# francois-rozet/sda

Hardware: AMD Instinct MI355X
Metric: diffusion-steps/s (Kolmogorov 64x256x256 posterior sampling; unit = one predictor-corrector step of a 16-trajectory per-GPU shard) (higher is better)
Workload: dtype f32; 1 GPU; kolmogorov256; per_gpu_batch=16, global_batch=16, guided=True, corrections=1, schedule_steps=1000, hipgraph_step=True, observation=fused Subsample (hand-written adjoint; no autograd through A), corrector_noise=row-keyed Philox (sda_randn_rows), parallelism=dp1 (batch-sharded, no in-loop collective), ranks_seen=1, process_group_live=False

## Files before the change

include/sda_hip.h:

```cpp
#ifndef SDA_HIP_H
#define SDA_HIP_H

#include <stdint.h>

#ifdef __cplusplus
extern "C" {
#endif

#define SDA_ABI_VERSION 13

enum {
    SDA_OK = 0,
    SDA_E_BADARG = -1,
    SDA_E_UNSUPPORTED = -2,
    SDA_E_LDS = -3
};

enum { SDA_ACT_NONE = 0, SDA_ACT_SILU = 1, SDA_ACT_RELU = 2, SDA_ACT_ELU = 3, SDA_ACT_GELU = 4, SDA_ACT_SELU = 5 };

int sda_abi_version(void);

typedef struct sda_conv_desc {
    const float* x;
    int64_t x_sn_outer, x_sn_inner;
    int32_t n_inner;
    int32_t x_n_off;
    int64_t x_sc, x_sy, x_sx;
    int32_t cx;
    const float* ctx;
    int64_t ctx_sn;
    int32_t cctx;
    int32_t n;
    int32_t hs, ws;
    int32_t up_h, up_w;
    int32_t zins_h, zins_w;
    const float* mod;
    int64_t mod_sn;
    const float* ln_mean;
    const float* ln_rstd;
    int32_t act_in;
    int32_t kh, kw, stride_h, stride_w, circular;
    const float* w;
    int32_t cin_pad, cout_pad;
    const float* bias;
    float* out;
    int32_t cout, ho, wo;
    const float* dact_z;
    int32_t act_d;
    const float* res;
    int32_t mt;
    const float* w_wino;
    int32_t explicit_pad, pad_h, pad_w;
    int64_t out_sn, out_sc, out_sy, out_sx;
    const float* w_wino4;
    int32_t pool_h, pool_w;
    const float* w_wino4_zp;
    const void* w_h2;
    float w_h2_scale;
    float x_amax_static;
    const float* x_amax;
    float* out_amax;
} sda_conv_desc;

int sda_conv_igemm(const sda_conv_desc* d, void* stream);
int sda_conv_parity4(const sda_conv_desc* d, void* stream);
int sda_conv_igemm_path(const sda_conv_desc* d);
int64_t sda_conv_igemm_lds_bytes(const sda_conv_desc* d);

typedef struct sda_block1d_desc {
    int32_t n, c, len;
    int32_t circular, act, unbiased;
    float eps;
    int32_t k_pad, m_pad;
    const float* a;
    const float* mod;
    int64_t mod_sn;
    const float* w1; const float* b1;
    const float* w2; const float* b2;
    float* z;
    float* mean; float* rstd;
    float* y;
    const float* g;
    float* gx;
} sda_block1d_desc;
int sda_block1d_fwd(const sda_block1d_desc* d, void* stream);
int sda_block1d_bwd(const sda_block1d_desc* d, void* stream);

#define SDA_NET1D_MAXB 8
typedef struct sda_net1d_desc {
    int32_t n, len;
    int32_t cin, c, cout;
    int32_t nblocks;
    int32_t circular, act, unbiased;
    float eps;
    const float* x; int64_t x_sn, x_sc, x_sx;
    float* out; int64_t out_sn, out_sc, out_sx;
    const float* w;
    const float* bias;
    const float* mod[SDA_NET1D_MAXB];
    int64_t mod_sn;
    float* a_save; float* z_save; int64_t save_stride;
    float* mean_save; float* rstd_save; int64_t stat_stride;
} sda_net1d_desc;
int sda_net1d_fwd(const sda_net1d_desc* d, void* stream);
int sda_net1d_bwd(const sda_net1d_desc* d, void* stream);

typedef struct sda_net1d_fuse {
    float cx0, cx1, cn;
    const float* coef;
    const float* y; int64_t y_sn;
    int32_t p_start, p_step, p_stop;
    int32_t c_start, c_step, c_stop;
    float std, gamma;
    float* ghat;
    const float* eps;
    int32_t mode;
    float* xs;
    const float* step_coef;
    float* partial; int32_t partial_stride;
} sda_net1d_fuse;
int sda_net1d_fwd_fused(const sda_net1d_desc* d, const sda_net1d_fuse* f, void* stream);
int sda_net1d_bwd_fused(const sda_net1d_desc* d, const sda_net1d_fuse* f, void* stream);
int sda_net1d_tiles(const sda_net1d_desc* d);

int sda_step1d_prologue(const float* table, int row_len, int64_t* istep, const float* t_dev, int nt,
                        int alpha_kind, float eta, float k, int sigma_kind,
                        const float* freqs, int nf, const float* w0, const float* b0, int hidden, const float* w2, const float* b2, int e,
                        const float* wp, const float* bp, int cp,
                        float* out_coef, int64_t* out_step, float* mod, void* stream);
int sda_pc_correct_keyed(float* x, const float* eps, int b, int64_t per_sample, const float* partial, int nchunk, float tau,
                         float sigma, const float* coef_dev, uint64_t seed, int64_t row0, const int64_t* draw_dev, int64_t draw_mul,
                         int64_t draw_add, void* stream);

int sda_pack_conv_weight(const float* w, int cout, int cin, int kh, int kw, int transpose, int cin_keep,
                         float* dst, int k_pad, int m_pad, void* stream);

int sda_pack_conv_weight_wino(const float* w, int cout, int cin, int transpose, int cin_keep, float* dst, int k_pad,
                              int m_pad, void* stream);

int sda_pack_conv_weight_wino4(const float* w, int cout, int cin, int transpose, int cin_keep, float* dst, int k_pad,
                               int m_pad, void* stream);
int sda_pack_conv_weight_wino4_zp(const float* w_wino4, int k_pad, int m_pad, float* dst, void* stream);
int64_t sda_wino4_zp_floats(int k_pad, int m_pad);

int sda_ln_stats(const float* x, int n, int c, int hw, const float* mod, int64_t mod_sn, float eps, int unbiased,
                 float* mean, float* rstd, void* stream);
int sda_ln_apply(const float* x, int n, int c, int hw, const float* mod, int64_t mod_sn, const float* mean,
                 const float* rstd, float* y, void* stream);
int sda_ln_bwd(const float* gh, const float* x, int n, int c, int h, int w, const float* mod, int64_t mod_sn,
               const float* mean, const float* rstd, int unbiased, int pool_h, int pool_w, const float* res, float* gx,
               void* stream);
int sda_ln_bwd_amax(const float* gh, const float* x, int n, int c, int h, int w, const float* mod, int64_t mod_sn,
                    const float* mean, const float* rstd, int unbiased, int pool_h, int pool_w, const float* res, float* gx,
                    float* amax, void* stream);

int sda_time_embed(const float* t, int nt, const float* freqs, int nf, const float* w0, const float* b0, int hidden,
                   const float* w2, const float* b2, int e, float* emb, void* stream);
int sda_linear_small(const float* x, int rows, int in_f, const float* w, const float* b, int out_f, float* y,
                     void* stream);

int sda_linear(const float* x, int rows, int in_f, const float* w, const float* b, int out_f, int trans_w, int act_in,
               int act_out, const float* dact_z, int act_d, const float* res, float* y, void* stream);
int sda_row_ln(const float* x, int rows, int f, float eps, int unbiased, float* y, float* mean, float* rstd, void* stream);
int sda_row_ln_bwd(const float* gh, const float* x, int rows, int f, const float* mean, const float* rstd, int unbiased,
                   const float* res, float* gx, void* stream);

#define SDA_MLP_MAXG 32
typedef struct sda_mlp_desc {
    int32_t rows, ngemm;
    int32_t act, unbiased;
    float eps;
    int32_t kind[SDA_MLP_MAXG];
    int32_t in_f[SDA_MLP_MAXG], out_f[SDA_MLP_MAXG];
    int32_t w_off[SDA_MLP_MAXG], b_off[SDA_MLP_MAXG];
    const float* w; const float* bias;
    const float* x; int64_t x_ld;
    float* out; int64_t out_ld;
    float* a_save; float* z_save; int64_t save_stride; int32_t save_ld;
    float* mean_save; float* rstd_save; int64_t stat_stride;
} sda_mlp_desc;
int sda_mlp_fwd(const sda_mlp_desc* d, void* stream);
int sda_mlp_bwd(const sda_mlp_desc* d, void* stream);
int sda_mlp_slab_floats(int in_f, int out_f);

typedef struct sda_mlp_win {
    int32_t nw, len, c, emb_n;
    const float* x; const float* emb;
    float cx0, cx1, cn;
    const float* coef;
    const float* y; int64_t y_sn;
    int32_t p_start, p_step, p_stop, c_start, c_step, c_stop;
    float std, gamma;
    float* eps; float* ghat;
    float* gwin;
} sda_mlp_win;
int sda_mlp_fwd_win(const sda_mlp_desc* d, const sda_mlp_win* w, void* stream);
// ... 84 lines not shown
```

sda_amd/_lib.py:

```python
import ctypes
import os
from ctypes import POINTER, Structure, c_float, c_int, c_int32, c_int64, c_uint32, c_uint64, c_void_p

import torch

HERE = os.path.dirname(os.path.abspath(__file__))
LIB_PATH = os.environ.get('SDA_HIP_LIB') or os.path.join(HERE, 'lib', 'libsda_hip.so')

ACT_IDS = {None: 0, 'none': 0, 'SiLU': 1, 'ReLU': 2, 'ELU': 3, 'GELU': 4, 'SELU': 5}

c_fp = c_void_p


class ConvDesc(Structure):
    _fields_ = [
        ('x', c_fp),
        ('x_sn_outer', c_int64), ('x_sn_inner', c_int64),
        ('n_inner', c_int32),
        ('x_n_off', c_int32),
        ('x_sc', c_int64), ('x_sy', c_int64), ('x_sx', c_int64),
        ('cx', c_int32),
        ('ctx', c_fp),
        ('ctx_sn', c_int64),
        ('cctx', c_int32),
# ... 94 lines not shown
        ('a_save', c_fp), ('z_save', c_fp), ('save_stride', c_int64), ('save_ld', c_int32),
        ('mean_save', c_fp), ('rstd_save', c_fp), ('stat_stride', c_int64),
    ]


class MlpWin(Structure):
    _fields_ = [
        ('nw', c_int32), ('len', c_int32), ('c', c_int32), ('emb_n', c_int32),
        ('x', c_fp), ('emb', c_fp),
        ('cx0', c_float), ('cx1', c_float), ('cn', c_float),
        ('coef', c_fp),
        ('y', c_fp), ('y_sn', c_int64),
        ('p_start', c_int32), ('p_step', c_int32), ('p_stop', c_int32),
        ('c_start', c_int32), ('c_step', c_int32), ('c_stop', c_int32),
        ('std', c_float), ('gamma', c_float),
        ('eps', c_fp), ('ghat', c_fp),
        ('gwin', c_fp),
    ]


class Net1dFuse(Structure):
    _fields_ = [
        ('cx0', c_float), ('cx1', c_float), ('cn', c_float),
        ('coef', c_fp),
        ('y', c_fp), ('y_sn', c_int64),
        ('p_start', c_int32), ('p_step', c_int32), ('p_stop', c_int32),
        ('c_start', c_int32), ('c_step', c_int32), ('c_stop', c_int32),
        ('std', c_float), ('gamma', c_float),
        ('ghat', c_fp),
        ('eps', c_fp),
        ('mode', c_int32),
        ('xs', c_fp),
        ('step_coef', c_fp),
        ('partial', c_fp), ('partial_stride', c_int32),
    ]


SIGNATURES = {
    'sda_abi_version': (c_int, []),
    'sda_conv_igemm': (c_int, [POINTER(ConvDesc), c_void_p]),
    'sda_gauss_cotangent': (c_int, [c_void_p, c_int64, c_void_p, c_int64, c_float, c_float, c_float, c_float, c_void_p, c_void_p, c_void_p]),
    'sda_block1d_fwd': (c_int, [POINTER(Block1dDesc), c_void_p]),
    'sda_block1d_bwd': (c_int, [POINTER(Block1dDesc), c_void_p]),
    'sda_net1d_fwd': (c_int, [POINTER(Net1dDesc), c_void_p]),
    'sda_net1d_bwd': (c_int, [POINTER(Net1dDesc), c_void_p]),
    'sda_net1d_fwd_fused': (c_int, [POINTER(Net1dDesc), POINTER(Net1dFuse), c_void_p]),
    'sda_net1d_bwd_fused': (c_int, [POINTER(Net1dDesc), POINTER(Net1dFuse), c_void_p]),
    'sda_net1d_tiles': (c_int, [POINTER(Net1dDesc)]),
    'sda_step1d_prologue': (c_int, [c_fp, c_int, c_fp, c_fp, c_int, c_int, c_float, c_float, c_int, c_fp, c_int, c_fp, c_fp, c_int,
                                    c_fp, c_fp, c_int, c_fp, c_fp, c_int, c_fp, c_fp, c_fp, c_void_p]),
    'sda_pc_correct_keyed': (c_int, [c_fp, c_fp, c_int, c_int64, c_fp, c_int, c_float, c_float, c_fp, c_uint64, c_int64, c_fp, c_int64,
                                     c_int64, c_void_p]),
    'sda_conv_parity4': (c_int, [POINTER(ConvDesc), c_void_p]),
    'sda_conv_igemm_path': (c_int, [POINTER(ConvDesc)]),
    'sda_conv_igemm_lds_bytes': (c_int64, [POINTER(ConvDesc)]),
    'sda_pack_conv_weight': (c_int, [c_fp, c_int, c_int, c_int, c_int, c_int, c_int, c_fp, c_int, c_int, c_void_p]),
    'sda_pack_conv_weight_wino': (c_int, [c_fp, c_int, c_int, c_int, c_int, c_fp, c_int, c_int, c_void_p]),
    'sda_pack_conv_weight_wino4': (c_int, [c_fp, c_int, c_int, c_int, c_int, c_fp, c_int, c_int, c_void_p]),
    'sda_pack_conv_weight_wino4_zp': (c_int, [c_fp, c_int, c_int, c_fp, c_void_p]),
    'sda_wino4_zp_floats': (c_int64, [c_int, c_int]),
    'sda_ln_stats': (c_int, [c_fp, c_int, c_int, c_int, c_fp, c_int64, c_float, c_int, c_fp, c_fp, c_void_p]),
    'sda_ln_apply': (c_int, [c_fp, c_int, c_int, c_int, c_fp, c_int64, c_fp, c_fp, c_fp, c_void_p]),
    'sda_ln_bwd': (c_int, [c_fp, c_fp, c_int, c_int, c_int, c_int, c_fp, c_int64, c_fp, c_fp, c_int, c_int, c_int, c_fp, c_fp,
                           c_void_p]),
    'sda_ln_bwd_amax': (c_int, [c_fp, c_fp, c_int, c_int, c_int, c_int, c_fp, c_int64, c_fp, c_fp, c_int, c_int, c_int, c_fp, c_fp,
                           c_fp, c_void_p]),
    'sda_time_embed': (c_int, [c_fp, c_int, c_fp, c_int, c_fp, c_fp, c_int, c_fp, c_fp, c_int, c_fp, c_void_p]),
    'sda_linear_small': (c_int, [c_fp, c_int, c_int, c_fp, c_fp, c_int, c_fp, c_void_p]),
    'sda_linear': (c_int, [c_fp, c_int, c_int, c_fp, c_fp, c_int, c_int, c_int, c_int, c_fp, c_int, c_fp, c_fp, c_void_p]),
    'sda_mlp_fwd': (c_int, [POINTER(MlpDesc), c_void_p]),
    'sda_mlp_bwd': (c_int, [POINTER(MlpDesc), c_void_p]),
    'sda_mlp_slab_floats': (c_int, [c_int, c_int]),
    'sda_mlp_fwd_win': (c_int, [POINTER(MlpDesc), POINTER(MlpWin), c_void_p]),
    'sda_mlp_bwd_win': (c_int, [POINTER(MlpDesc), POINTER(MlpWin), c_void_p]),
    'sda_mc_finish': (c_int, [c_fp, c_fp, c_fp, c_int, c_int, c_int, c_int, c_float, c_float, c_fp, c_int, c_fp, c_fp, c_fp, c_fp, c_void_p]),
    'sda_row_ln': (c_int, [c_fp, c_int, c_int, c_float, c_int, c_fp, c_fp, c_fp, c_void_p]),
    'sda_row_ln_bwd': (c_int, [c_fp, c_fp, c_int, c_int, c_fp, c_fp, c_int, c_fp, c_fp, c_void_p]),
    'sda_obs_subsample': (c_int, [c_fp, POINTER(c_int), POINTER(c_int), POINTER(c_int), POINTER(c_int), c_fp, c_void_p]),
    'sda_obs_subsample_adjoint': (c_int, [c_fp, POINTER(c_int), POINTER(c_int), POINTER(c_int), POINTER(c_int), c_fp, c_void_p]),
    'sda_obs_pointwise': (c_int, [c_fp, c_int64, c_int, c_fp, c_void_p]),
    'sda_obs_pointwise_vjp': (c_int, [c_fp, c_fp, c_int64, c_int, c_fp, c_void_p]),
    'sda_obs_mask': (c_int, [c_fp, c_int64, c_fp, c_int64, c_fp, c_void_p]),
    'sda_obs_timediff': (c_int, [c_fp, c_int64, c_int, c_int64, c_int, c_int, c_fp, c_void_p]),
    'sda_obs_timediff_adjoint': (c_int, [c_fp, c_int64, c_int, c_int64, c_int, c_int, c_fp, c_void_p]),
    'sda_obs_subsample_guidance': (c_int, [c_fp, c_fp, c_fp, c_int64, POINTER(c_int), POINTER(c_int), POINTER(c_int), POINTER(c_int),
                                           c_float, c_float, c_float, c_float, c_fp, c_fp, c_void_p]),
    'sda_obs_coarsen': (c_int, [c_fp, c_int64, c_int, c_int, c_int, c_fp, c_void_p]),
    'sda_obs_coarsen_adjoint': (c_int, [c_fp, c_int64, c_int, c_int, c_int, c_fp, c_void_p]),
    'sda_obs_vorticity': (c_int, [c_fp, c_int64, c_int, c_int, c_fp, c_void_p]),
    'sda_obs_vorticity_adjoint': (c_int, [c_fp, c_int64, c_int, c_int, c_fp, c_void_p]),
    'sda_fold': (c_int, [c_fp, c_int, c_int, c_int, c_int, c_int, c_fp, c_void_p]),
    'sda_fold_adjoint': (c_int, [c_fp, c_int, c_int, c_int, c_int, c_int, c_fp, c_void_p]),
    'sda_unfold_adjoint': (c_int, [c_fp, c_int, c_int, c_int, c_int, c_int, c_int64, c_fp, c_void_p]),
    'sda_vp_schedule': (c_int, [c_fp, c_int, c_float, c_float, c_int, c_fp, c_void_p]),
    'sda_pc_predict': (c_int, [c_fp, c_fp, c_int64, c_float, c_float, c_fp, c_void_p]),
    'sda_sumsq_partial': (c_int, [c_fp, c_int, c_int64, c_fp, c_int, c_void_p]),
    'sda_pc_correct': (c_int, [c_fp, c_fp, c_fp, c_int, c_int64, c_fp, c_int, c_float, c_float, c_fp, c_void_p]),
    'sda_randn_rows': (c_int, [c_fp, c_int, c_int64, c_uint64, c_int64, c_int64, c_fp, c_int64, c_int64, c_void_p]),
    'sda_clock_probe': (c_int, [c_void_p, c_int, c_void_p, c_int, c_void_p]),
    'sda_conv_h2': (c_int, [POINTER(ConvDesc), c_void_p]),
    'sda_conv_h2_supported': (c_int, [POINTER(ConvDesc)]),
    'sda_pack_conv_weight_h2': (c_int, [c_fp, c_int, c_int, c_int, c_float, c_void_p, c_void_p]),
    'sda_conv_h2_packed_bytes': (c_int64, [c_int, c_int, c_int]),
    'sda_pack_conv_weight_h2_up': (c_int, [c_fp, c_int, c_int, c_float, c_void_p, c_void_p]),
    'sda_conv_h2_up_packed_bytes': (c_int64, [c_int, c_int]),
    'sda_pack_conv_weight_h2_rows': (c_int, [c_fp, c_int, c_int, c_int, c_float, c_void_p, c_void_p]),
# ... 54 lines not shown
```

sda_amd/build.py:

```python
import hashlib
import os
import subprocess
import sys

HERE = os.path.dirname(os.path.abspath(__file__))
CSRC = os.path.join(HERE, 'csrc')
LIBDIR = os.environ.get('SDA_LIBDIR') or os.path.join(HERE, 'lib')
ARCH = 'gfx950'
SOURCES = ['conv_igemm.hip', 'conv_wino.hip', 'conv_wino4.hip', 'conv_small1d.hip', 'conv_few.hip', 'conv_par4.hip', 'conv_h2.hip', 'conv3d.hip', 'block1d.hip', 'net1d.hip', 'step1d.hip', 'norm.hip', 'elementwise.hip', 'linear.hip', 'mlp1d.hip', 'observe.hip', 'metrics.hip', 'noise.hip', 'probe.hip']
HIPCC = os.environ.get('HIPCC', '/opt/rocm/bin/hipcc')
EXTRA_FLAGS = os.environ.get('SDA_EXTRA_HIPCC_FLAGS', '').split()
CONV_PARTS = 4


def _digest(deps, flags=()):
    h = hashlib.sha256()
    for d in deps:
        h.update(os.path.basename(d).encode())
        with open(d, 'rb') as f:
            h.update(f.read())
    h.update(' '.join(flags).encode())
    return h.hexdigest()


def _newer(target, deps, flags=()):
    stamp = target + '.stamp'
    if not os.path.exists(target) or not os.path.exists(stamp):
        return True
    with open(stamp) as f:
        return f.read().strip() != _digest(deps, flags)


def _stamp(target, deps, flags=()):
    with open(target + '.stamp', 'w') as f:
        f.write(_digest(deps, flags))


def _headers():
    hs = [os.path.join(CSRC, f) for f in os.listdir(CSRC) if f.endswith('.hpp')]
    hs.append(os.path.join(os.path.dirname(HERE), 'include', 'sda_hip.h'))
    return hs


def build(force=False, verbose=False):
    os.makedirs(LIBDIR, exist_ok=True)
    objs = []
    hdrs = _headers()
    procs = []
    units = []
    for src in SOURCES:
        if src == 'conv_igemm.hip':
            units += [(src, f'_p{k}', [f'-DSDA_CONV_PART={k}']) for k in range(CONV_PARTS)]
        else:
            units.append((src, '', []))
    for src, suffix, flags in units:
        sp = os.path.join(CSRC, src)
        if not os.path.exists(sp):
            continue
        obj = os.path.join(LIBDIR, src.replace('.hip', suffix + '.o'))
        objs.append(obj)
        cflags = ['-O3', '-std=c++17', '-fPIC', '-ffp-contract=off'] + flags + EXTRA_FLAGS
        if force or _newer(obj, [sp] + hdrs, cflags):
# ... 37 lines not shown
```

sda_amd/engine.py:

```python
import math
from dataclasses import dataclass
from typing import List, Optional

import torch
import torch.nn as nn
from torch import Tensor

from . import ops
from ._lib import SdaHipError
from .ops import PackedConv, conv_out_size, make_conv_desc


def _lib_net1d_maxb() -> int:
    from ._lib import NET1D_MAXB
    return NET1D_MAXB


def _net1d_span_ok(sc: int, sx: int, channels: int, length: int) -> bool:
    return sc >= 0 and sx >= 0 and sc * channels + sx * length < 1 << 30


CHUNK_HBM_FRACTION = 0.45
KEEP_HBM_FRACTION = 0.45
PARITY_SPLIT = True
# ... 8 lines not shown
    hs: int
    ws: int
    sn_outer: int
    sc: int
    sy: int
    sx: int
    sn_inner: int = 0
    n_inner: int = 1
    ctx: Optional[Tensor] = None
    cctx: int = 0
    ctx_sn: int = 0


def planar_source(a: Tensor) -> dict:
    n, c, h, w = a.shape
    return dict(x_ptr=a.data_ptr(), n=n, cx=c, hs=h, ws=w, x_sn_outer=c * h * w, x_sc=h * w, x_sy=w, x_sx=1)


class _ConvCache:

    def __init__(self, conv: nn.Module):
        if conv.dilation != (1,) * len(conv.dilation) or conv.groups != 1:
            raise NotImplementedError('dilated / grouped convolutions have no gfx950 kernel')
        if conv.padding_mode not in ('zeros', 'circular'):
            raise NotImplementedError(f"padding_mode={conv.padding_mode!r} (supported: 'zeros', 'circular')")
        ks = conv.kernel_size
        if any(k % 2 == 0 for k in ks):
            raise NotImplementedError('even kernel sizes are not supported')
        self.conv = conv
        self.kh, self.kw = (1, ks[0]) if len(ks) == 1 else ks
        st = conv.stride
        self.sh, self.sw = (1, st[0]) if len(st) == 1 else st
        self.circular = conv.padding_mode == 'circular'
        self.cin, self.cout = conv.in_channels, conv.out_channels
        self._key = None
        self._fwd = None
        self._bwd = {}
        self._parity = None

    def _sync(self):
        w = self.conv.weight
        key = (w.data_ptr(), ops.tensor_version(w), str(w.device), None if self.conv.bias is None else ops.tensor_version(self.conv.bias),
               ops.MULTIPLY)
        if key != self._key:
            self._key, self._fwd, self._bwd, self._parity = key, None, {}, None

    def invalidate(self):
        self._key = None

    def fwd(self) -> PackedConv:
        self._sync()
        if self._fwd is None:
            self._fwd = PackedConv(self.conv.weight, self.conv.bias, transpose=False)
        return self._fwd

    def bwd(self, cin_keep: Optional[int] = None) -> PackedConv:
        self._sync()
        if cin_keep not in self._bwd:
            self._bwd[cin_keep] = PackedConv(self.conv.weight, None, transpose=True, cin_keep=cin_keep)
        return self._bwd[cin_keep]

    def bwd_parity(self):
        self._sync()
        if self._parity is None:
            taps = []
            for k, s in ((self.kh, self.sh), (self.kw, self.sw)):
                if s == 1:
                    taps.append([(None, list(range(k)), k // 2)])
                elif s == 2 and k == 3:
                    taps.append([(0, [1], 0), (1, [0, 2], 0)])
                else:
                    taps = None
                    break
            if taps is None or (self.sh == 1 and self.sw == 1):
                self._parity = False
            else:
                w = self.conv.weight.detach()
                if w.dim() == 3:
                    w = w.unsqueeze(2)
                out = []
                for py, ty, ph in taps[0]:
                    for px, tx, pw in taps[1]:
                        sub = w[:, :, ty][:, :, :, tx].contiguous()
                        out.append((py, px, PackedConv(sub, None, transpose=True), (ph, pw)))
                self._parity = out
        return self._parity or None

    def bwd_parity4(self):
        classes = self.bwd_parity()
        if not classes or len(classes) != 4 or [(py, px) for py, px, _, _ in classes] != [(0, 0), (0, 1), (1, 0), (1, 1)]:
            return None
        if getattr(self, '_parity4', None) is None or self._parity4[0] is not classes:
            pks = [pk for _, _, pk, _ in classes]
            if any(pk.k_pad != pks[0].k_pad or pk.m_pad != pks[0].m_pad or pk.m_pad != pk.m_real for pk in pks):
                return None
            self._parity4 = (classes, torch.cat([pk.packed for pk in pks]))
        return self._parity4[1]


def launch_conv(pk: PackedConv, src: dict, out: Tensor, ho: int, wo: int, *, circular: bool, stride=(1, 1), up=(1, 1),
                zins=(1, 1), bias: Optional[Tensor] = None, mod: Optional[Tensor] = None, mod_sn: int = 0,
                ln=None, act_in: int = 0, dact_z: Optional[Tensor] = None, act_d: int = 0, res: Optional[Tensor] = None,
                ctx: Optional[Tensor] = None, cctx: int = 0, ctx_sn: int = 0, pad=None, parity4_w: Optional[Tensor] = None,
                pool=(1, 1), x_amax=None, out_amax: Optional[Tensor] = None, h2_only: bool = False):
    out_strides = (0, 0, 0, 0)
    if not out.is_contiguous():
        out_strides = tuple(out.stride())
        for t in (dact_z, res):
            if t is not None and tuple(t.stride()) != out_strides:
                raise SdaHipError('conv epilogue operands must share the layout of the output view')
    zp = pk.wino4_zp() if (tuple(up) == (2, 2) or tuple(pool) == (2, 2)) and hasattr(pk, 'wino4_zp') else None
    d = make_conv_desc(**src, w_ptr=pk.packed.data_ptr(), cin_pad=pk.k_pad, cout_pad=pk.m_pad, cout=pk.m_real,
                       kh=pk.kh, kw=pk.kw, out_ptr=out.data_ptr(), ho=ho, wo=wo, mt=pk.mt,
                       stride_h=stride[0], stride_w=stride[1], circular=circular, up_h=up[0], up_w=up[1],
                       zins_h=zins[0], zins_w=zins[1],
                       ctx_ptr=None if ctx is None else ctx.data_ptr(), cctx=cctx, ctx_sn=ctx_sn,
                       mod_ptr=None if mod is None else mod.data_ptr(), mod_sn=mod_sn,
                       ln_mean_ptr=None if ln is None else ln[0].data_ptr(),
                       ln_rstd_ptr=None if ln is None else ln[1].data_ptr(),
                       act_in=act_in, bias_ptr=None if bias is None else bias.data_ptr(),
                       dact_z_ptr=None if dact_z is None else dact_z.data_ptr(), act_d=act_d,
                       res_ptr=None if res is None else res.data_ptr(),
                       w_wino_ptr=None if getattr(pk, 'wino', None) is None else pk.wino.data_ptr(),
                       w_wino4_ptr=None if getattr(pk, 'wino4', None) is None else pk.wino4.data_ptr(),
                       pad=pad, out_strides=out_strides, pool=pool, w_wino4_zp_ptr=None if zp is None else zp.data_ptr())
    if pool != (1, 1):
        if tuple(pool) == (2, 2) and ops.H2_POOL and x_amax is not None and getattr(pk, 'h2', None) is not None:
            packing = pk.h2_pool()
            if packing is not None and ops.conv_h2(d, pk, x_amax, out_amax, packing=packing):
                return d
        return d if ops.conv_pooled(d) else None
    if getattr(pk, 'h2', None) is not None and parity4_w is None:
        bound = math.sqrt(src['cx']) if ln is not None else x_amax
        packing = None
        if tuple(up) == (2, 2):
            packing = pk.h2_up() if ops.H2_UP else None
            if packing is None:
                bound = None
        elif tuple(zins) == (2, 2) or tuple(stride) == (2, 2):
            packing = (pk.h2_zins() if tuple(zins) == (2, 2) else pk.h2_s2()) if ops.H2_S2 else None
            if packing is None:
                bound = None
        if ops.conv_h2(d, pk, bound, out_amax, packing=packing):
            return d
    if h2_only:
        return None
    if parity4_w is not None:
        d.w = parity4_w.data_ptr()
        d.kh = d.kw = 2
        return d if ops.conv_parity4(d) else None
    ops.conv_igemm(d)
    return d


class _Block:
    def __init__(self, block, width: int, mod_off: int):
        from .nn import LayerNorm, activation_id
        residue = block.residue
        if not (len(residue) == 4 and isinstance(residue[0], LayerNorm)):
            raise NotImplementedError('unexpected residue structure')
        self.ln = residue[0]
        self.conv1 = _ConvCache(residue[1])
        self.act = activation_id(residue[2])
        self.conv2 = _ConvCache(residue[3])
        self.project = block.project[0]
        self.width = width
        self.mod_off = mod_off


class _Level:
    pass


class UNetEngine:
    def __init__(self, unet):
        from .nn import LN_UNBIASED
        if unet.spatial not in (1, 2):
            raise NotImplementedError('this engine serves spatial = 1, 2 (spatial = 3: engine3d.UNet3dEngine)')
        self.unet = unet
        self.unbiased = LN_UNBIASED
        self.depth = len(unet.hidden_blocks)
        D = self.depth
        self.levels: List[_Level] = []
        off = 0
        for lvl in range(D):
            lev = _Level()
            lev.C = unet.hidden_channels[lvl]
            j = D - 1 - lvl
            head = unet.heads[lvl] if lvl == 0 else unet.heads[lvl][0]
            lev.head = _ConvCache(head)
            if lvl == 0:
                lev.tail = _ConvCache(unet.tails[j])
                lev.tail_ln = None
            else:
                lev.tail_ln = unet.tails[j][0]
                lev.tail = _ConvCache(unet.tails[j][2])
            lev.descent, lev.ascent = [], []
            for blk in unet.descent[lvl]:
                lev.descent.append(_Block(blk, lev.C, off)); off += lev.C
            for blk in unet.ascent[j]:
                lev.ascent.append(_Block(blk, lev.C, off)); off += lev.C
            self.levels.append(lev)
        self.mod_total = off
# ... 551 lines not shown
```

sda_amd/ops.py:

```python
import ctypes
import math
import os
from typing import Optional

import torch
from torch import Tensor

from . import _lib
from ._lib import ACT_IDS, ConvDesc

CONV_CK = 8
WINOGRAD = os.environ.get('SDA_CONV_WINO', '1') != '0'
WINOGRAD4 = os.environ.get('SDA_CONV_WINO4', '1') != '0'
MULTIPLY = os.environ.get('SDA_MULTIPLY', 'f32')
if MULTIPLY not in ('f32', 'f16x2'):
    raise ValueError(f"SDA_MULTIPLY={MULTIPLY!r} (expected 'f32' or 'f16x2')")


def set_multiply(mode: str) -> str:
    global MULTIPLY
    if mode not in ('f32', 'f16x2'):
        raise ValueError(f"multiply mode {mode!r} (expected 'f32' or 'f16x2')")
    prev, MULTIPLY = MULTIPLY, mode
    return prev
# ... 165 lines not shown
    if packing is None:
        desc.w_h2, desc.w_h2_scale = pk.h2.data_ptr(), pk.h2_scale
    else:
        desc.w_h2, desc.w_h2_scale = packing[0].data_ptr(), packing[1]
    if torch.is_tensor(x_amax):
        desc.x_amax, desc.x_amax_static = x_amax.data_ptr(), 0.0
    else:
        desc.x_amax, desc.x_amax_static = None, float(x_amax)
    desc.out_amax = None if out_amax is None else out_amax.data_ptr()
    if not lib.sda_conv_h2_supported(ctypes.byref(desc)):
        desc.w_h2 = None
        return False
    prof = conv_profile
    if prof is not None:
        e0, e1 = torch.cuda.Event(enable_timing=True), torch.cuda.Event(enable_timing=True)
        e0.record()
    if out_amax is not None:
        out_amax.zero_()
    _lib.check(lib.sda_conv_h2(ctypes.byref(desc), _stream()), 'sda_conv_h2')
    if prof is not None:
        e1.record()
        fam = 'h2up' if (desc.up_h == 2 or desc.pool_h == 2) else 'h2s2' if (desc.zins_h == 2 or desc.stride_h == 2) else 'h2'
        prof.records.append((e0, e1, prof.flops(desc) / float(max(1, desc.zins_h) * max(1, desc.zins_w)), fam))
        rd, wr = prof.alg_bytes(desc)
        b = prof.family_bytes.setdefault(fam, [0.0, 0.0])
        b[0] += rd
        b[1] += wr
    return True


PARITY4 = os.environ.get('SDA_CONV_PAR4', '1') != '0'
WINO4_BM64 = os.environ.get('SDA_W4_BM64', '1') != '0'


def conv_parity4(desc: ConvDesc) -> bool:
    lib = _lib.load()
    prof = conv_profile
    if prof is not None:
        e0, e1 = torch.cuda.Event(enable_timing=True), torch.cuda.Event(enable_timing=True)
        e0.record()
    rc = lib.sda_conv_parity4(ctypes.byref(desc), _stream())
    if rc == -2:
        return False
    _lib.check(rc, 'sda_conv_parity4')
    if prof is not None:
        e1.record()
        prof.records.append((e0, e1, 2.0 * desc.n * desc.ho * desc.wo * desc.cout * desc.cx * 9, 'par4'))
        b = prof.family_bytes.setdefault('par4', [0.0, 0.0])
        b[0] += 4.0 * desc.n * desc.cx * desc.hs * desc.ws + 4.0 * 9 * desc.cx * desc.cout + (16.0 * desc.n * desc.cout * desc.ho * desc.wo if desc.res else 0.0)
        b[1] += 16.0 * desc.n * desc.cout * desc.ho * desc.wo
    return True


POOLED = os.environ.get('SDA_CONV_POOLED', '1') != '0'


def conv_pooled(desc: ConvDesc) -> bool:
    lib = _lib.load()
    if lib.sda_conv_igemm_path(ctypes.byref(desc)) < 0:
        return False
    conv_igemm(desc)
    return True


CONV_FAMILIES = ('direct', 'wino', 'wino4', 'small1d', 'few', 'wino4zp')


def conv_path(desc: ConvDesc) -> int:
    return _lib.load().sda_conv_igemm_path(ctypes.byref(desc))


def pack_conv_weight(w: Tensor, cout: int, cin: int, kh: int, kw: int, transpose: bool, keep: int, dst: Tensor,
                     k_pad: int, m_pad: int):
    _lib.check(_lib.load().sda_pack_conv_weight(w.data_ptr(), cout, cin, kh, kw, int(transpose), keep, dst.data_ptr(),
                                                k_pad, m_pad, _stream()), 'sda_pack_conv_weight')


class PackedConv:

    def __init__(self, weight: Tensor, bias: Optional[Tensor], transpose: bool = False, cin_keep: Optional[int] = None):
        _dev(weight, bias)
        w = weight.detach().contiguous()
        cout, cin = w.shape[0], w.shape[1]
        ks = tuple(w.shape[2:])
        self.kh, self.kw = (1, ks[0]) if len(ks) == 1 else ks
        self._transpose = bool(transpose)
        self._w_ref = w if (MULTIPLY == 'f16x2' and len(ks) == 2) else None
        self._h2_up = None
        self._h2_pool = None
        self._h2_zins = None
        self._h2_s2 = None
        if transpose:
            keep = cin if cin_keep is None else cin_keep
            self.k_real, self.m_real = cout, keep
        else:
            keep = cin
            self.k_real, self.m_real = cin, cout
        self.mt = pick_mt(self.m_real)
        self.k_pad = round_up(self.k_real, CONV_CK)
        self.m_pad = round_up(self.m_real, 32 * self.mt)
        self.packed = torch.empty(self.kh * self.kw * self.k_pad * self.m_pad, device=w.device, dtype=torch.float32)
        pack_conv_weight(w, cout, cin, self.kh, self.kw, transpose, keep, self.packed, self.k_pad, self.m_pad)
        self.bias = None if (bias is None or transpose) else bias.detach().contiguous()
        self.wino = None
        if WINOGRAD and (self.kh, self.kw) == (3, 3) and self.m_real % 96 == 0 and self.mt == 3:
            self.wino = torch.empty(16 * self.k_pad * self.m_pad, device=w.device, dtype=torch.float32)
            _lib.check(_lib.load().sda_pack_conv_weight_wino(w.data_ptr(), cout, cin, int(transpose), keep,
                                                             self.wino.data_ptr(), self.k_pad, self.m_pad, _stream()),
                       'sda_pack_conv_weight_wino')
        self.wino4 = None
        if WINOGRAD4 and (self.kh, self.kw) == (3, 3) and self.m_pad == self.m_real and (self.wino is not None or (WINO4_BM64 and self.m_real % 32 == 0)):
            self.wino4 = torch.empty(16 * self.k_pad * self.m_pad, device=w.device, dtype=torch.float32)
            _lib.check(_lib.load().sda_pack_conv_weight_wino4(w.data_ptr(), cout, cin, int(transpose), keep,
                                                              self.wino4.data_ptr(), self.k_pad, self.m_pad, _stream()),
                       'sda_pack_conv_weight_wino4')
        self._wino4_zp = None
        if self.wino4 is not None:
            lib = _lib.load()
            self._wino4_zp = torch.empty(int(lib.sda_wino4_zp_floats(self.k_pad, self.m_pad)), device=w.device, dtype=torch.float32)
            _lib.check(lib.sda_pack_conv_weight_wino4_zp(self.wino4.data_ptr(), self.k_pad, self.m_pad, self._wino4_zp.data_ptr(), _stream()),
                       'sda_pack_conv_weight_wino4_zp')

        self.h2 = None
        if MULTIPLY == 'f16x2' and (self.kh, self.kw) == (3, 3) and (not transpose or keep == cin) and w.numel() > 0:
            lib = _lib.load()
            nbytes = int(lib.sda_conv_h2_packed_bytes(cout, cin, int(transpose)))
            if nbytes > 0:
                w_amax = float(w.abs().max())
                if w_amax > 0.0 and math.isfinite(w_amax):
                    self.h2 = torch.empty(nbytes, device=w.device, dtype=torch.uint8)
                    _lib.check(lib.sda_pack_conv_weight_h2(w.data_ptr(), cout, cin, int(transpose), w_amax, self.h2.data_ptr(), _stream()),
                               'sda_pack_conv_weight_h2')
                    self.h2_scale = float(lib.sda_conv_h2_scale(w_amax))
                    self.out_amax = torch.zeros(1, device=w.device, dtype=torch.float32)
                    self.in_amax = torch.zeros(1, device=w.device, dtype=torch.float32)

    def _h2_wsum(self) -> Tensor:
        w = self._w_ref
        cout, cin = w.shape[0], w.shape[1]
        rows = (((0,), (1, 2)), ((0, 1), (2,)))
        wsum = torch.empty(4, cout, cin, 4, device=w.device, dtype=torch.float32)
        for py in range(2):
            for px in range(2):
                for a_ in range(2):
                    for b_ in range(2):
                        acc = None
                        for dy in rows[py][a_]:
                            for dx in rows[px][b_]:
                                acc = w[:, :, dy, dx] if acc is None else acc + w[:, :, dy, dx]
                        wsum[2 * py + px, :, :, 2 * a_ + b_] = acc
        return wsum

    def h2_up(self):
        if self.h2 is None or self._transpose or getattr(self, '_w_ref', None) is None:
            return None
        if getattr(self, '_h2_up', None) is None:
            lib = _lib.load()
            cout, cin = self._w_ref.shape[0], self._w_ref.shape[1]
            nbytes = int(lib.sda_conv_h2_up_packed_bytes(cout, cin))
            self._h2_up = False
            if nbytes > 0:
                wsum = self._h2_wsum()
# ... 485 lines not shown
```

Before: 0.1378 diffusion-steps/s.

## Add Winograd-style kernel for stride-2 3x3 forward convolutions

Adds a HIP kernel that computes stride-2 3x3 convolutions through a 5x5 transformed-input product, with weights pre-transformed into 25 positions at pack time. Producer waves stage transformed input and weight slabs into double-buffered LDS while consumer waves run f32 MFMA accumulations, and the epilogue folds the results into 2x2 outputs. The aim is to cut the multiply count and the im2col-style overhead of the generic igemm path for downsampling convolutions. It costs an extra packed weight buffer and applies only when the channel counts and spatial sizes are aligned; the different summation order can change rounding.

```diff
diff --git a/include/sda_hip.h b/include/sda_hip.h
--- a/include/sda_hip.h
+++ b/include/sda_hip.h
@@ -64,6 +64,8 @@
 
 int sda_conv_igemm(const sda_conv_desc* d, void* stream);
 int sda_conv_parity4(const sda_conv_desc* d, void* stream);
+int sda_conv_s2w(const sda_conv_desc* d, void* stream);
+int sda_conv_s2w_supported(const sda_conv_desc* d);
 int sda_conv_igemm_path(const sda_conv_desc* d);
 int64_t sda_conv_igemm_lds_bytes(const sda_conv_desc* d);
 
@@ -142,6 +144,7 @@
                                int m_pad, void* stream);
 int sda_pack_conv_weight_wino4_zp(const float* w_wino4, int k_pad, int m_pad, float* dst, void* stream);
 int64_t sda_wino4_zp_floats(int k_pad, int m_pad);
+int sda_pack_conv_weight_s2w(const float* w, int cout, int cin, float* dst, int k_pad, int m_pad, void* stream);
 
 int sda_ln_stats(const float* x, int n, int c, int hw, const float* mod, int64_t mod_sn, float eps, int unbiased,
                  float* mean, float* rstd, void* stream);
diff --git a/sda_amd/_lib.py b/sda_amd/_lib.py
--- a/sda_amd/_lib.py
+++ b/sda_amd/_lib.py
@@ -170,6 +170,9 @@
     'sda_pc_correct_keyed': (c_int, [c_fp, c_fp, c_int, c_int64, c_fp, c_int, c_float, c_float, c_fp, c_uint64, c_int64, c_fp, c_int64,
                                      c_int64, c_void_p]),
     'sda_conv_parity4': (c_int, [POINTER(ConvDesc), c_void_p]),
+    'sda_conv_s2w': (c_int, [POINTER(ConvDesc), c_void_p]),
+    'sda_conv_s2w_supported': (c_int, [POINTER(ConvDesc)]),
+    'sda_pack_conv_weight_s2w': (c_int, [c_fp, c_int, c_int, c_fp, c_int, c_int, c_void_p]),
     'sda_conv_igemm_path': (c_int, [POINTER(ConvDesc)]),
     'sda_conv_igemm_lds_bytes': (c_int64, [POINTER(ConvDesc)]),
     'sda_pack_conv_weight': (c_int, [c_fp, c_int, c_int, c_int, c_int, c_int, c_int, c_fp, c_int, c_int, c_void_p]),
diff --git a/sda_amd/build.py b/sda_amd/build.py
--- a/sda_amd/build.py
+++ b/sda_amd/build.py
@@ -7,7 +7,7 @@
 CSRC = os.path.join(HERE, 'csrc')
 LIBDIR = os.environ.get('SDA_LIBDIR') or os.path.join(HERE, 'lib')
 ARCH = 'gfx950'
-SOURCES = ['conv_igemm.hip', 'conv_wino.hip', 'conv_wino4.hip', 'conv_small1d.hip', 'conv_few.hip', 'conv_par4.hip', 'conv_h2.hip', 'conv3d.hip', 'block1d.hip', 'net1d.hip', 'step1d.hip', 'norm.hip', 'elementwise.hip', 'linear.hip', 'mlp1d.hip', 'observe.hip', 'metrics.hip', 'noise.hip', 'probe.hip']
+SOURCES = ['conv_igemm.hip', 'conv_wino.hip', 'conv_wino4.hip', 'conv_small1d.hip', 'conv_few.hip', 'conv_par4.hip', 'conv_s2w.hip', 'conv_h2.hip', 'conv3d.hip', 'block1d.hip', 'net1d.hip', 'step1d.hip', 'norm.hip', 'elementwise.hip', 'linear.hip', 'mlp1d.hip', 'observe.hip', 'metrics.hip', 'noise.hip', 'probe.hip']
 HIPCC = os.environ.get('HIPCC', '/opt/rocm/bin/hipcc')
 EXTRA_FLAGS = os.environ.get('SDA_EXTRA_HIPCC_FLAGS', '').split()
 CONV_PARTS = 4
diff --git a/sda_amd/csrc/conv_s2w.hip b/sda_amd/csrc/conv_s2w.hip
--- /dev/null
+++ b/sda_amd/csrc/conv_s2w.hip
@@ -0,0 +1,236 @@
+#include "sda_common.hpp"
+#include <stdlib.h>
+
+#define SW_CK 4
+#define SW_TBY 4
+#define SW_TBX 16
+#define SW_NB (SW_TBY * SW_TBX)
+#define SW_BM 64
+#define SW_SLAB (25 * SW_CK * SW_BM)
+#define SW_BUF (2 * SW_SLAB)
+#define SW_NU ((SW_SLAB / 4 + 255) / 256)
+
+typedef float sw_f32x16 __attribute__((ext_vector_type(16)));
+typedef float sw_f32x4 __attribute__((ext_vector_type(4)));
+typedef float sw_f32x2 __attribute__((ext_vector_type(2)));
+
+__device__ constexpr int SW_AM[5] = {0, 1, 0, 2, 1};
+
+template <bool CIRC>
+__global__ __launch_bounds__(512, 2) void conv_s2w_kernel(const sda_conv_desc d, int tiles_x, int tiles_y, int n_ct) {
+    extern __shared__ __attribute__((aligned(16))) float smem[];
+    const int tid = threadIdx.x, lane = tid & 63, l31 = lane & 31, khalf = lane >> 5;
+    const int wave = __builtin_amdgcn_readfirstlane(tid >> 6);
+    int t;
+    {
+        const int total = (int)gridDim.x, xcd = (int)blockIdx.x & 7, slot = (int)blockIdx.x >> 3;
+        const int tq = total >> 3, tr = total & 7;
+        t = xcd * tq + (xcd < tr ? xcd : tr) + slot;
+    }
+    const int ct = t % n_ct; t /= n_ct;
+    const int bx = t % tiles_x; t /= tiles_x;
+    const int by = t % tiles_y;
+    const int n = t / tiles_y;
+    const int oy0 = by * (2 * SW_TBY), ox0 = bx * (2 * SW_TBX), co0 = ct * SW_BM;
+    const int nstage = d.cin_pad / SW_CK;
+    if (wave >= 4) {
+        const int ptid = tid - 256;
+        const int kh = ptid & 1, blk = (ptid >> 1) & 63, kp = ptid >> 7;
+        const int ch = 2 * kp + kh;
+        const int bry = blk / SW_TBX, brx = blk - bry * SW_TBX;
+        const float* ximg = d.x + (int64_t)n * d.x_sn_outer;
+        const int fy0 = 2 * (oy0 + 2 * bry), fx0 = 2 * (ox0 + 2 * brx);
+        const int ym = fy0 > 0 ? fy0 - 1 : (CIRC ? d.hs - 1 : 0);
+        const int xm = fx0 > 0 ? fx0 - 1 : (CIRC ? d.ws - 1 : 0);
+        const bool ylive = CIRC || fy0 > 0, xlive = CIRC || fx0 > 0;
+        unsigned off4[5], off1[5];
+#pragma unroll
+        for (int r = 0; r < 5; ++r) {
+            const int ro = ch * (int)d.x_sc + (r == 0 ? ym : fy0 - 1 + r) * (int)d.x_sy;
+            off4[r] = (unsigned)(ro + fx0);
+            off1[r] = (unsigned)(ro + xm);
+        }
+        unsigned uoff[SW_NU];
+#pragma unroll
+        for (int i = 0; i < SW_NU; ++i) {
+            const int f = ptid + 256 * i;
+            const int pos = f >> 6, kq = (f >> 5) & 1, c = f & 31;
+            uoff[i] = (unsigned)(((pos * (d.cin_pad >> 1) + kq) * d.cout_pad + co0) * 2 + 4 * c);
+        }
+        sw_f32x4 rv4[5];
+        float rv1[5];
+        sw_f32x4 uv[SW_NU];
+        const auto rsx = __builtin_amdgcn_make_buffer_rsrc(const_cast<float*>(ximg), (short)0, (int)((int64_t)d.cx * d.x_sc * 4), 0x00020000);
+        const auto rsu = __builtin_amdgcn_make_buffer_rsrc(const_cast<float*>(d.w), (short)0, (int)((int64_t)25 * d.cin_pad * d.cout_pad * 4),
+                                                          0x00020000);
+        auto load = [&](int st) {
+            const int sx = st * SW_CK * (int)d.x_sc * 4, su = st * SW_CK * d.cout_pad * 4;
+#pragma unroll
+            for (int r = 0; r < 5; ++r) {
+                rv4[r] = __builtin_bit_cast(sw_f32x4, __builtin_amdgcn_raw_buffer_load_b128(rsx, (int)(off4[r] * 4), sx, 0));
+                rv1[r] = __builtin_bit_cast(float, __builtin_amdgcn_raw_buffer_load_b32(rsx, (int)(off1[r] * 4), sx, 0));
+            }
+#pragma unroll
+            for (int i = 0; i < SW_NU; ++i)
+                if (i + 1 < SW_NU || ptid + 256 * i < SW_SLAB / 4)
+                    uv[i] = __builtin_bit_cast(sw_f32x4, __builtin_amdgcn_raw_buffer_load_b128(rsu, (int)(uoff[i] * 4), su, 0));
+        };
+        auto store = [&](float* buf) {
+            sw_f32x2 row[5][3];
+#pragma unroll
+            for (int r = 0; r < 5; ++r) {
+                const float a0 = (xlive && (ylive || r > 0)) ? rv1[r] : 0.f;
+                sw_f32x4 v = rv4[r];
+                if (!CIRC && r == 0 && !ylive) v = sw_f32x4{0.f, 0.f, 0.f, 0.f};
+                row[r][0] = sw_f32x2{v[0], v[2]};
+                row[r][1] = sw_f32x2{a0, v[3]} - sw_f32x2{v[1], v[1]};
+                row[r][2] = sw_f32x2{v[1], v[1]};
+            }
+            auto rx = [&](int r, int j) -> float {
+                return j == 0 ? row[r][0][0] : j == 1 ? row[r][0][1] : j == 2 ? row[r][1][0] : j == 3 ? row[r][2][0] : row[r][1][1];
+            };
+            float* vb = buf + ptid;
+#pragma unroll
+            for (int j = 0; j < 5; ++j) {
+                const sw_f32x2 m = sw_f32x2{rx(0, j), rx(4, j)} - sw_f32x2{rx(2, j), rx(2, j)};
+                vb[(5 * 0 + j) * 256] = rx(1, j);
+                vb[(5 * 1 + j) * 256] = rx(3, j);
+                vb[(5 * 2 + j) * 256] = m[0];
+                vb[(5 * 3 + j) * 256] = rx(2, j);
+                vb[(5 * 4 + j) * 256] = m[1];
+            }
+            float* ub = buf + SW_SLAB;
+#pragma unroll
+            for (int i = 0; i < SW_NU; ++i) {
+                const int f = ptid + 256 * i;
+                if (i + 1 < SW_NU || f < SW_SLAB / 4) *reinterpret_cast<sw_f32x4*>(ub + 4 * f) = uv[i];
+            }
+        };
+        load(0);
+        store(smem);
+        if (nstage > 1) load(1);
+        __syncthreads();
+        for (int st = 0; st < nstage; ++st) {
+            if (st + 1 < nstage) {
+                store(smem + ((st + 1) & 1) * SW_BUF);
+                if (st + 2 < nstage) load(st + 2);
+            }
+            __syncthreads();
+        }
+        return;
+    }
+    const int wm = wave & 1, wn = wave >> 1;
+    sw_f32x16 acc[9];
+#pragma unroll
+    for (int s = 0; s < 9; ++s)
+#pragma unroll
+        for (int r = 0; r < 16; ++r) acc[s][r] = 0.f;
+    const int bbase = 2 * (32 * wn + l31) + khalf;
+    const int abase = SW_SLAB + 2 * (32 * wm + l31) + khalf;
+    __syncthreads();
+    for (int st = 0; st < nstage; ++st) {
+        const float* buf = smem + (st & 1) * SW_BUF;
+#pragma unroll
+        for (int kq = 0; kq < SW_CK / 2; ++kq) {
+#pragma unroll
+            for (int pos = 0; pos < 25; ++pos) {
+                const float a = buf[abase + pos * 256 + kq * 128];
+                const float b = buf[bbase + pos * 256 + kq * 128];
+                const int s = 3 * SW_AM[pos / 5] + SW_AM[pos % 5];
+                acc[s] = __builtin_amdgcn_mfma_f32_32x32x2f32(a, b, acc[s], 0, 0, 0);
+            }
+        }
+        __syncthreads();
+    }
+    const int blk = 32 * wn + l31, bry = blk / SW_TBX, brx = blk - bry * SW_TBX;
+    const int oy = oy0 + 2 * bry, ox = ox0 + 2 * brx;
+    const int64_t hw = (int64_t)d.ho * d.wo;
+    float* obase = d.out + (int64_t)n * d.cout * hw + (int64_t)oy * d.wo + ox;
+    const int cbase = co0 + 32 * wm + 4 * khalf;
+#pragma unroll
+    for (int r = 0; r < 16; ++r) {
+        const int co = cbase + (r & 3) + 8 * (r >> 2);
+        const float bias = d.bias ? d.bias[co] : 0.f;
+        float* o = obase + (int64_t)co * hw;
+#pragma unroll
+        for (int py = 0; py < 2; ++py) {
+            const float r0 = acc[3 * py + 0][r] + acc[6 + 0][r];
+            const float r1 = acc[3 * py + 1][r] + acc[6 + 1][r];
+            const float rm = acc[3 * py + 2][r] + acc[6 + 2][r];
+            const sw_f32x2 v = sw_f32x2{r0 + rm, r1 + rm} + sw_f32x2{bias, bias};
+            *reinterpret_cast<sw_f32x2*>(o + py * d.wo) = v;
+        }
+    }
+}
+
+static bool s2w_ok(const sda_conv_desc* d) {
+    if (!d || !d->x || !d->w || !d->out) return false;
+    if (d->kh != 3 || d->kw != 3 || d->stride_h != 2 || d->stride_w != 2 || d->explicit_pad || d->up_h != 1 || d->up_w != 1 ||
+        d->zins_h != 1 || d->zins_w != 1 || (d->pool_h > 1) || (d->pool_w > 1))
+        return false;
+    if (d->cctx != 0 || d->mod || d->ln_mean || d->ln_rstd || d->act_in != SDA_ACT_NONE || d->dact_z || d->res || d->n_inner != 1 ||
+        d->x_n_off != 0 || d->out_sn || d->out_sc || d->out_sy || d->out_sx)
+        return false;
+    if ((d->cout % SW_BM) || d->cout_pad != d->cout || d->cin_pad % SW_CK || d->cx != d->cin_pad) return false;
+    if (d->hs != 2 * d->ho || d->ws != 2 * d->wo || (d->ho % (2 * SW_TBY)) || (d->wo % (2 * SW_TBX))) return false;
+    if (d->x_sx != 1 || d->x_sy < d->ws || (d->x_sy & 3) || (d->x_sc & 3) || (d->x_sn_outer & 3) ||
+        (reinterpret_cast<uintptr_t>(d->x) & 15) || (reinterpret_cast<uintptr_t>(d->w) & 15) || (reinterpret_cast<uintptr_t>(d->out) & 7))
+        return false;
+    if (d->x_sc < (int64_t)d->hs * d->x_sy || (int64_t)d->cx * d->x_sc * 4 >= (1LL << 31)) return false;
+    if ((int64_t)25 * d->cin_pad * d->cout_pad * 4 >= (1LL << 31)) return false;
+    const int64_t tiles = (int64_t)d->n * (d->ho / (2 * SW_TBY)) * (d->wo / (2 * SW_TBX)) * (d->cout / SW_BM);
+    return d->n >= 1 && tiles >= 1 && tiles <= 0x7fffffffLL;
+}
+
+template <bool CIRC>
+static int s2w_launch(const sda_conv_desc* d, hipStream_t stream) {
+    static bool attr_set[SDA_MAX_DEVICES];
+    const int lds = 2 * SW_BUF * 4;
+    const int rc = sda_raise_dyn_lds(reinterpret_cast<const void*>(conv_s2w_kernel<CIRC>), lds, attr_set);
+    if (rc != SDA_OK) return rc;
+    const int tx = d->wo / (2 * SW_TBX), ty = d->ho / (2 * SW_TBY), n_ct = d->cout / SW_BM;
+    hipLaunchKernelGGL(conv_s2w_kernel<CIRC>, dim3((unsigned)((int64_t)d->n * tx * ty * n_ct)), dim3(512), (size_t)lds, stream, *d, tx, ty,
+                       n_ct);
+    return sda_launch_status();
+}
+
+extern "C" int sda_conv_s2w_supported(const sda_conv_desc* d) { return s2w_ok(d) ? 1 : 0; }
+
+extern "C" int sda_conv_s2w(const sda_conv_desc* d, void* stream) {
+    if (!s2w_ok(d)) return SDA_E_UNSUPPORTED;
+    return d->circular ? s2w_launch<true>(d, (hipStream_t)stream) : s2w_launch<false>(d, (hipStream_t)stream);
+}
+
+__global__ void pack_s2w_kernel(const float* __restrict__ w, int cout, int cin, float* __restrict__ dst, int k_pad, int m_pad) {
+    const int64_t total = (int64_t)25 * k_pad * m_pad;
+    for (int64_t e = (int64_t)blockIdx.x * blockDim.x + threadIdx.x; e < total; e += (int64_t)gridDim.x * blockDim.x) {
+        const int h = (int)(e & 1);
+        int64_t r = e >> 1;
+        const int co = (int)(r % m_pad);
+        r /= m_pad;
+        const int kq = (int)(r % (k_pad / 2));
+        const int pos = (int)(r / (k_pad / 2));
+        const int ci = 2 * kq + h, i = pos / 5, j = pos % 5;
+        float v = 0.f;
+        if (ci < cin && co < cout) {
+            const float* g = w + ((int64_t)co * cin + ci) * 9;
+            float rowv[3];
+#pragma unroll
+            for (int ky = 0; ky < 3; ++ky) {
+                const float* gr = g + 3 * ky;
+                rowv[ky] = (j == 0 || j == 1) ? gr[1] : j == 2 ? gr[0] : j == 3 ? gr[0] + gr[2] : gr[2];
+            }
+            v = (i == 0 || i == 1) ? rowv[1] : i == 2 ? rowv[0] : i == 3 ? rowv[0] + rowv[2] : rowv[2];
+        }
+        dst[e] = v;
+    }
+}
+
+extern "C" int sda_pack_conv_weight_s2w(const float* w, int cout, int cin, float* dst, int k_pad, int m_pad, void* stream) {
+    if (!w || !dst || cout <= 0 || cin <= 0 || k_pad < cin || m_pad < cout || (k_pad & 1)) return SDA_E_BADARG;
+    const int64_t total = (int64_t)25 * k_pad * m_pad;
+    int blocks = (int)((total + 255) / 256);
+    if (blocks > 4096) blocks = 4096;
+    hipLaunchKernelGGL(pack_s2w_kernel, dim3(blocks), dim3(256), 0, (hipStream_t)stream, w, cout, cin, dst, k_pad, m_pad);
+    return sda_launch_status();
+}
diff --git a/sda_amd/engine.py b/sda_amd/engine.py
--- a/sda_amd/engine.py
+++ b/sda_amd/engine.py
@@ -84,6 +84,9 @@
         self._sync()
         if self._fwd is None:
             self._fwd = PackedConv(self.conv.weight, self.conv.bias, transpose=False)
+            if ops.S2W and (self.kh, self.kw, self.sh, self.sw) == (3, 3, 2, 2) and self._fwd.m_real % 64 == 0 and \
+                    self._fwd.m_pad == self._fwd.m_real and self._fwd.k_pad % 4 == 0:
+                self._fwd.s2w = ops.pack_conv_weight_s2w(self.conv.weight, self._fwd.k_pad, self._fwd.m_pad)
         return self._fwd
 
     def bwd(self, cin_keep: Optional[int] = None) -> PackedConv:
@@ -181,6 +184,8 @@
         d.w = parity4_w.data_ptr()
         d.kh = d.kw = 2
         return d if ops.conv_parity4(d) else None
+    if getattr(pk, 's2w', None) is not None and ops.conv_s2w(d, pk.s2w):
+        return d
     ops.conv_igemm(d)
     return d
 
diff --git a/sda_amd/ops.py b/sda_amd/ops.py
--- a/sda_amd/ops.py
+++ b/sda_amd/ops.py
@@ -241,6 +241,40 @@
     return True
 
 
+S2W = os.environ.get('SDA_CONV_S2W', '1') != '0'
+
+
+def pack_conv_weight_s2w(w: Tensor, k_pad: int, m_pad: int) -> Tensor:
+    _dev(w)
+    w = w.detach().contiguous()
+    dst = torch.empty(25 * k_pad * m_pad, device=w.device, dtype=torch.float32)
+    _lib.check(_lib.load().sda_pack_conv_weight_s2w(w.data_ptr(), w.shape[0], w.shape[1], dst.data_ptr(), k_pad, m_pad, _stream()),
+               'sda_pack_conv_weight_s2w')
+    return dst
+
+
+def conv_s2w(desc: ConvDesc, w_s2w: Tensor) -> bool:
+    lib = _lib.load()
+    w_direct = desc.w
+    desc.w = w_s2w.data_ptr()
+    if not lib.sda_conv_s2w_supported(ctypes.byref(desc)):
+        desc.w = w_direct
+        return False
+    prof = conv_profile
+    if prof is not None:
+        e0, e1 = torch.cuda.Event(enable_timing=True), torch.cuda.Event(enable_timing=True)
+        e0.record()
+    _lib.check(lib.sda_conv_s2w(ctypes.byref(desc), _stream()), 'sda_conv_s2w')
+    if prof is not None:
+        e1.record()
+        prof.records.append((e0, e1, prof.flops(desc), 's2w'))
+        rd, wr = prof.alg_bytes(desc)
+        b = prof.family_bytes.setdefault('s2w', [0.0, 0.0])
+        b[0] += rd
+        b[1] += wr
+    return True
+
+
 POOLED = os.environ.get('SDA_CONV_POOLED', '1') != '0'
 
 
@@ -297,6 +331,7 @@
             _lib.check(_lib.load().sda_pack_conv_weight_wino(w.data_ptr(), cout, cin, int(transpose), keep,
                                                              self.wino.data_ptr(), self.k_pad, self.m_pad, _stream()),
                        'sda_pack_conv_weight_wino')
+        self.s2w = None
         self.wino4 = None
         if WINOGRAD4 and (self.kh, self.kw) == (3, 3) and self.m_pad == self.m_real and (self.wino is not None or (WINO4_BM64 and self.m_real % 32 == 0)):
             self.wino4 = torch.empty(16 * self.k_pad * self.m_pad, device=w.device, dtype=torch.float32)
```

Result: no change. 0.1384 diffusion-steps/s, median of 6 (+0.4%).
